# Vandermode/ELD

Measured on AMD Instinct MI355X. Metric: raw megapixels/sec (noise-synth + U-Net step), higher is better.
Workload: dtype f32; 1 GPU; BASELINE.json configs[1]: full ELD noise model (PGRU, SonyA7S2 params) on 4x1424x2128 packed raw + U-Net fp32 train step (fwd, L1, bwd, Adam), 8 frames per GPU; images_per_gpu=8, global_batch=8, parallelism=dp1

## Files before the change

eld_amd/csrc/conv.h:

```cpp
#pragma once
#include "common.h"

typedef float f32x16 __attribute__((ext_vector_type(16)));
typedef float f32x2 __attribute__((ext_vector_type(2)));
typedef __bf16 bf16x2_hw __attribute__((ext_vector_type(2)));

enum ConvMode { CONV_3X3 = 0, CONV_1X1 = 1, CONV_GATHER2X2 = 2 };
enum ConvEpi { EPI_FWD = 0, EPI_CONVT_FWD = 1, EPI_GRAD = 2 };

typedef unsigned short bf16_t;
enum ConvDtype { DT_F32 = 0, DT_BF16 = 1 };

struct ConvArgs {
    const void* in0;
    const void* in1;
    int C0, C1;
    const void* wp;
    int N, H, W;
    int Nout;
    int epi;
    const float* bias;
    int lrelu;
    void* out0;
    void* out1;
// ... 148 lines not shown
__device__ __forceinline__ void eld_wait_vmcnt() { asm volatile("s_waitcnt vmcnt(%0)" ::"n"(N) : "memory"); }
__device__ __forceinline__ void eld_wait_vmcnt_dyn(int n) {
    switch (n) {
#define ELD_W(k) case k: eld_wait_vmcnt<k>(); break;
        ELD_W(1) ELD_W(2) ELD_W(3) ELD_W(4) ELD_W(5) ELD_W(6) ELD_W(7) ELD_W(8) ELD_W(9) ELD_W(10) ELD_W(11) ELD_W(12) ELD_W(13) ELD_W(14) ELD_W(15) ELD_W(16)
        ELD_W(17) ELD_W(18) ELD_W(19) ELD_W(20) ELD_W(21) ELD_W(22) ELD_W(23) ELD_W(24) ELD_W(25) ELD_W(26) ELD_W(27) ELD_W(28) ELD_W(29) ELD_W(30) ELD_W(31) ELD_W(32)
        ELD_W(33) ELD_W(34) ELD_W(35) ELD_W(36) ELD_W(37) ELD_W(38) ELD_W(39) ELD_W(40) ELD_W(41) ELD_W(42) ELD_W(43) ELD_W(44) ELD_W(45) ELD_W(46) ELD_W(47) ELD_W(48)
#undef ELD_W
        default: eld_wait_vmcnt<0>(); break;
    }
}

__device__ __forceinline__ void f32_rows_swap(float4& a, float4& b) {
    auto r = __builtin_amdgcn_permlane16_swap(__float_as_uint(a.x), __float_as_uint(b.x), false, false); a.x = __uint_as_float(r[0]); b.x = __uint_as_float(r[1]);
    r = __builtin_amdgcn_permlane16_swap(__float_as_uint(a.y), __float_as_uint(b.y), false, false); a.y = __uint_as_float(r[0]); b.y = __uint_as_float(r[1]);
    r = __builtin_amdgcn_permlane16_swap(__float_as_uint(a.z), __float_as_uint(b.z), false, false); a.z = __uint_as_float(r[0]); b.z = __uint_as_float(r[1]);
    r = __builtin_amdgcn_permlane16_swap(__float_as_uint(a.w), __float_as_uint(b.w), false, false); a.w = __uint_as_float(r[0]); b.w = __uint_as_float(r[1]);
}
__device__ __forceinline__ void st16(float* p, float4 v, bool wt = false) {
    typedef float f4v __attribute__((ext_vector_type(4)));
    const f4v q = {v.x, v.y, v.z, v.w};
    if (wt) asm volatile("global_store_dwordx4 %0, %1, off sc1" ::"v"(p), "v"(q) : "memory");
    else *reinterpret_cast<float4*>(p) = v;
}
__device__ __forceinline__ void f32_line_store(float4 (&v)[4], float* blk, size_t pstride, int lane, bool row_ok, int valid_px, bool wt = false) {
    f32_rows_swap(v[0], v[1]);
    f32_rows_swap(v[2], v[3]);
    const int lp = lane & 15;
    float* p0 = blk + (size_t)lp * pstride + 4 * bf16_line_group(lane);
    if (row_ok && lp < valid_px) {
        st16(p0, v[0], wt);
        st16(p0 + 16, v[2], wt);
    }
    if (row_ok && lp + 16 < valid_px) {
        float* p1 = p0 + 16 * pstride;
        st16(p1, v[1], wt);
        st16(p1 + 16, v[3], wt);
    }
}

__host__ __device__ inline int vrow_extent(int N, int H, int P) { return (N - 1) * P + H; }
__host__ __device__ inline int vrow_pitch(int N, int H, int TH) {
    const int flat = H + 2 - (H & 1), own = (H + TH - 1) / TH * TH;
    if (flat < TH + 2) return own;
    return (vrow_extent(N, H, flat) + TH - 1) / TH < (vrow_extent(N, H, own) + TH - 1) / TH ? flat : own;
}

void conv_tile_shape(int N, int H, int W, int TH, bool pooled, int& th, int& tw);
__host__ __device__ inline int conv_slot_of_lane(int m, bool grouped) {
    if (!grouped) return m;
    const int q = m >> 2;
    const int sq = q == 0 ? 0 : q == 1 ? 4 : q == 2 ? 5 : q == 3 ? 1 : q == 4 ? 6 : q == 5 ? 2 : q == 6 ? 3 : 7;
    return sq * 4 + (m & 3);
}
__host__ __device__ inline bool conv_slots_grouped(int th, int tw, int TH) { return !(th == TH && tw == 32); }
long long conv_tile_count(int N, int H, int W, int TH, bool pooled);
const char* conv_tile_variant();

__device__ __forceinline__ void f32_line_store2(float4 (&v)[4], float* p0, float* p1, int lane, bool wt = false) {
    f32_rows_swap(v[0], v[1]);
    f32_rows_swap(v[2], v[3]);
    const int g = 4 * bf16_line_group(lane);
    if (p0 != nullptr) {
        st16(p0 + g, v[0], wt);
        st16(p0 + g + 16, v[2], wt);
    }
    if (p1 != nullptr) {
        st16(p1 + g, v[1], wt);
        st16(p1 + g + 16, v[3], wt);
    }
}

int launch_conv(const ConvArgs& a, int mode, hipStream_t st);
int conv_fp32_algo(int set);
inline int resolve_algo(int algo) { return (algo >= 0 && algo <= 2) ? algo : conv_fp32_algo(-1); }
int launch_conv_x3(const ConvArgs& a, hipStream_t st);
int x3_slab_bn(int Nout, int N, int H, int W, int* waves = nullptr);
__host__ __device__ inline size_t x3_slab_stride(int BN) { return (size_t)(3 * BN * 112 + 1023) / 1024 * 1024; }
void conv_x3_set_prof(unsigned long long* buf);
int launch_conv_x3_gemm(const ConvArgs& a, int mode, hipStream_t st);
bool x3w_enabled();
bool x3w_takes(const ConvArgs& a);
int launch_conv_x3w(const ConvArgs& a, hipStream_t st);
int bfd_slab_bn(int Nout, int K, int N, int H, int W);
__host__ __device__ inline size_t bfd_slab_bytes(int BN) { return (size_t)3 * BN * 64; }
int launch_conv_bfd(const ConvArgs& a, hipStream_t st);
int debug_kernel_mask(int set);
bool bfs_takes(int Nout, int K, int N, int H, int W);
int launch_conv_bfs(const ConvArgs& a, hipStream_t st);
bool bfw_takes(const ConvArgs& a);
int launch_conv_bfw(const ConvArgs& a, hipStream_t st);
int bfg_slab_bn(bool gather, int Nout, int Cs, int Cout_t, int N, int H, int W);
__host__ __device__ inline size_t bfg_slab_bytes(int BN) { return (size_t)BN * 64; }
int launch_conv_bfg(const ConvArgs& a, int mode, hipStream_t st);

#ifdef __HIPCC__
__device__ __forceinline__ int xcd_block(int on) {
    const int b = (int)blockIdx.x;
    if (!on) return b;
    const int n = (int)gridDim.x, q = n >> 3, r = n & 7, x = b & 7;
    return (x < r ? x * (q + 1) : r * (q + 1) + (x - r) * q) + (b >> 3);
}
#endif
__host__ __device__ inline void band_tile(int id, int tiles_x, int tiles_y, int BH, int& ty, int& tx) {
    if (BH <= 1) { ty = id / tiles_x; tx = id - ty * tiles_x; return; }
    const int full = tiles_x * BH, band = id / full, off = id - band * full;
    int bh = tiles_y - band * BH;
    if (bh > BH) bh = BH;
    tx = off / bh;
    ty = band * BH + (off - tx * bh);
}
int eld_tile_band();
enum { XCD_GEMM = 1, XCD_WGRAD8 = 2, XCD_WGRAD = 4, XCD_X3D = 8, XCD_X3W = 16, XCD_BF16 = 32, XCD_IGEMM = 64 };
int eld_xcd_mask();

struct WgradArgs {
    const void* g;
    int CA;
    const void* x0;
    const void* x1;
    int C0, C1;
    int N, H, W;
    float* part;
    float* bpart;
    float* xbpart;
    int CBp;
    int psplit;
    int tiles_x, tiles_y;
    int vp;
    int dtype;
    int algo;
    int wgrad8;
    int xcd;
    int band;
    const float* amax_g; const float* amax_x0; const float* amax_x1;
};

int launch_wgrad(const WgradArgs& a, int mode, hipStream_t st);
bool wgrad8_shape(int CA, int CBp, int& COB, int& JB, int& TH, int& TWo, bool bf16 = false);
int wgrad8_ntiles(int CA, int CBp, int N, int H, int W, bool bf16);
bool wgradt8_takes(int CA, int CB);
int wgradt8_ntiles(int N, int H, int W);
int launch_wgrad_reduce(const float* part, const float* bpart, float* wgrad, float* bgrad, int psplit, int T, int CA,
                        int CBp, int CBr, hipStream_t st, int bias_n = 0);
```

eld_amd/csrc/conv_x3.hip:

```cpp
#include <stdlib.h>
#include "conv.h"

#include "conv_x3_dev.h"

namespace {

template <int BN, int RPW, bool DB, bool BFIRST = false, bool BSLAB = false, bool STREAM = false>
__global__ __launch_bounds__(256, 2) void conv_x3_kernel(const ConvArgs a) {
    constexpr int CK = 16;
    constexpr int TH = 4 * RPW, NT = BN / 32, A_PIX = (TH + 2) * (TW + 2);
    constexpr int A_WORDS = A_PIX * PX, B_ROWS = 3 * BN;
    extern __shared__ __attribute__((aligned(16))) float lds[];
    float* ldsA = lds;
    float* ldsB = lds + A_WORDS;

    const int tid = threadIdx.x, lane = tid & 63, wave = tid >> 6;
    const int m = lane & 31, hi = lane >> 5;
    const int NB = a.Nout / BN;
    const int Cin = a.C0 + a.C1;
    const int total_tiles = a.tiles_x * a.tiles_y * a.N * NB;
    const int Cs0 = a.C0;

    constexpr int A_UNITS = A_PIX * 4, B_UNITS = BSLAB ? B_ROWS * 7 : B_ROWS * 4;
    constexpr int A_IT = (A_UNITS + 255) / 256, B_IT = (B_UNITS + 255) / 256;
// ... 813 lines not shown
    }
}

template <bool POOL>
__global__ __launch_bounds__(256) void x3_splitk_finish_kernel(const ConvArgs a) {
    const int Q = a.Nout >> 2;
    const int Wb = POOL ? a.W >> 1 : a.W, Hb = POOL ? a.H >> 1 : a.H;
    const size_t total = (size_t)a.N * Hb * Wb * Q;
    const size_t plane = (size_t)a.N * a.H * a.W * a.Nout;
    for (size_t i = (size_t)blockIdx.x * 256 + threadIdx.x; i < total; i += (size_t)gridDim.x * 256) {
        const int q = (int)(i % Q);
        size_t p = i / Q;
        const int xb = (int)(p % Wb); p /= Wb;
        const int yb = (int)(p % Hb);
        const int img = (int)(p / Hb);
        const int n = 4 * q;
        float4 pooled = make_float4(0.f, 0.f, 0.f, 0.f);
#pragma unroll
        for (int w = 0; w < (POOL ? 4 : 1); ++w) {
            const int y = POOL ? 2 * yb + (w >> 1) : yb, x = POOL ? 2 * xb + (w & 1) : xb;
            const size_t pix = (size_t)(img * a.H + y) * a.W + x;
            float4 v = make_float4(0.f, 0.f, 0.f, 0.f);
            for (int ks = 0; ks < a.ksplit; ++ks) {
                const float4 t = *reinterpret_cast<const float4*>(a.kpart + (size_t)ks * plane + pix * a.Nout + n);
                v.x += t.x; v.y += t.y; v.z += t.z; v.w += t.w;
            }
            if (a.epi == EPI_FWD) {
                const float4 b = *reinterpret_cast<const float4*>(a.bias + n);
                v.x += b.x; v.y += b.y; v.z += b.z; v.w += b.w;
                if (a.lrelu) { v.x = fmaxf(0.2f * v.x, v.x); v.y = fmaxf(0.2f * v.y, v.y); v.z = fmaxf(0.2f * v.z, v.z); v.w = fmaxf(0.2f * v.w, v.w); }
                *reinterpret_cast<float4*>(static_cast<float*>(a.out0) + pix * a.Nout + n) = v;
                if (POOL) pooled = w == 0 ? v : make_float4(fmaxf(pooled.x, v.x), fmaxf(pooled.y, v.y), fmaxf(pooled.z, v.z), fmaxf(pooled.w, v.w));
            } else {
                const bool lo = n < a.split;
                const int C = lo ? a.split : a.Nout - a.split;
                const size_t idx = pix * C + (lo ? n : n - a.split);
                const float* act = static_cast<const float*>(lo ? a.act0 : a.act1);
                if (act) {
                    const float4 s_ = *reinterpret_cast<const float4*>(act + idx);
                    v.x *= lrelu_slope(s_.x); v.y *= lrelu_slope(s_.y); v.z *= lrelu_slope(s_.z); v.w *= lrelu_slope(s_.w);
                }
                *reinterpret_cast<float4*>(static_cast<float*>(lo ? a.out0 : a.out1) + idx) = v;
            }
        }
        if (POOL) *reinterpret_cast<float4*>(static_cast<float*>(a.pool_out) + ((size_t)(img * Hb + yb) * Wb + xb) * a.Nout + n) = pooled;
    }
}

int launch_x3_splitk_finish(const ConvArgs& a, hipStream_t st) {
    const bool pool = a.epi == EPI_FWD && a.pool_out != nullptr;
    const size_t total = (size_t)a.N * (pool ? a.H / 2 : a.H) * (pool ? a.W / 2 : a.W) * (a.Nout / 4);
    if (!total) return 0;
    const unsigned grid = (unsigned)((total + 255) / 256 < 4096 ? (total + 255) / 256 : 4096);
    if (pool) { ELD_LAUNCH(x3_splitk_finish_kernel<true>, dim3(grid), dim3(256), 0, st, a); }
    else { ELD_LAUNCH(x3_splitk_finish_kernel<false>, dim3(grid), dim3(256), 0, st, a); }
    ELD_LAUNCH_CHECK();
    return 0;
}

template <int BN, int RPW, bool DB, bool BFIRST = false, bool BSLAB = false, bool STREAM = false>
int launch_x3(ConvArgs a, hipStream_t st) {
    a.xcd = eld_xcd_mask() & XCD_X3W;
    constexpr int TH = 4 * RPW;
    a.tiles_x = (a.W + TW - 1) / TW;
    a.tiles_y = (a.H + TH - 1) / TH;
    const size_t lds_bytes = (size_t)((TH + 2) * (TW + 2) + 3 * BN) * PX * sizeof(float);
    const long long tiles = (long long)a.tiles_x * a.tiles_y * a.N * (a.Nout / BN);
    if (tiles <= 0) return 0;
    if (tiles > 0x7fffffffLL) return ELD_ENOTSUP;
    eld_note_conv_variant("conv_x3<32>", BSLAB ? nullptr : "cut", BFIRST ? nullptr : "bfirst0", STREAM ? nullptr : "stream0");
    auto kern = conv_x3_kernel<BN, RPW, DB, BFIRST, BSLAB, STREAM>;
    static EldAttrOnce once;
    { const int rc = once.ensure(kern, lds_bytes); if (rc) return rc; }
    int per_cu = (int)((160 * 1024) / lds_bytes);
    if (per_cu > 2) per_cu = 2;
    if (per_cu < 1 || (ELD_DBG(a) & 64)) per_cu = 1;
    long long grid = (long long)eld_num_cus() * per_cu;
    if (grid > tiles) grid = tiles;
    ELD_LAUNCH(kern, dim3((unsigned)grid), dim3(256), lds_bytes, st, a);
    ELD_LAUNCH_CHECK();
    return 0;
}

template <int BN, int RPW, int WAVES, bool DB, int STREAM = 0>
int launch_x3d(ConvArgs a, hipStream_t st) {
    a.xcd = eld_xcd_mask() & XCD_X3D;
    constexpr int TH = WAVES * RPW;
    conv_tile_shape(a.N, a.H, a.W, TH, a.pool_out != nullptr, a.tile_h, a.tile_w);
    a.vp = vrow_pitch(a.N, a.H, a.tile_h);
    a.tiles_x = (a.W + a.tile_w - 1) / a.tile_w;
    a.tiles_y = (vrow_extent(a.N, a.H, a.vp) + a.tile_h - 1) / a.tile_h;
    const size_t lds_bytes = (size_t)(TH + 2) * (TW + 2) * PX * sizeof(float) + 2 * (size_t)((3 * BN * PX * 4 + 1023) / 1024 * 1024);
    long long tiles = (long long)a.tiles_x * a.tiles_y * (a.Nout / BN);
    if (tiles <= 0) return 0;
    a.ksplit = 1;
    static const int no_splitk = [] { const char* e = getenv("ELD_NO_SPLITK"); return e ? atoi(e) : 0; }();
    if (WAVES == 4 && a.kpart != nullptr && !no_splitk) {
        const int nch = (a.C0 + a.C1) / 16;
        const size_t plane = (size_t)a.N * a.H * a.W * a.Nout;
        int ks = (int)(eld_num_cus() / tiles);
        if (ks > nch / 2) ks = nch / 2;
        if (ks > 16) ks = 16;
        while (ks > 1 && (size_t)ks * plane > a.kpart_floats) --ks;
        if (ks >= 2) { a.ksplit = ks; tiles *= ks; }
    }
    if (tiles > 0x7fffffffLL) return ELD_ENOTSUP;
    eld_note_conv_variant(BN == 128 ? "conv_x3d<128,8>" : (BN == 32 ? "conv_x3d<32,8>" : (WAVES == 8 ? "conv_x3d<64,8>" : (a.ksplit > 1 ? "conv_x3d<64,4,splitk>" : "conv_x3d<64,4>"))),
                          (WAVES == 8 && BN >= 64) ? (STREAM == 0 ? "stream0" : (STREAM == 1 ? "wreuse0" : nullptr)) : nullptr,
                          a.pool_out ? nullptr : conv_tile_variant());
    auto kern = conv_x3d_kernel<BN, RPW, WAVES, DB, STREAM>;
    static EldAttrOnce once;
    { const int rc = once.ensure(kern, lds_bytes); if (rc) return rc; }
    int per_cu = (int)((160 * 1024) / lds_bytes);
    if (per_cu > 2) per_cu = 2;
    if (per_cu < 1) per_cu = 1;
    long long grid = (long long)eld_num_cus() * per_cu;
    if (grid > tiles) grid = tiles;
    ELD_LAUNCH(kern, dim3((unsigned)grid), dim3(64 * WAVES), lds_bytes, st, a);
    ELD_LAUNCH_CHECK();
    if (a.ksplit > 1) return launch_x3_splitk_finish(a, st);
    return 0;
}

template <int MODE, int BN, int WAVES>
int launch_x3_gemm(ConvArgs a, hipStream_t st) {
    a.xcd = eld_xcd_mask() & XCD_GEMM;
    constexpr int TH = 2 * WAVES;
    a.tiles_x = (a.W + TW - 1) / TW;
    a.tiles_y = (a.H + TH - 1) / TH;
    const size_t lds_bytes = (size_t)(2 * TH * TW + 2 * BN) * PX * sizeof(float);
    const long long tiles = (long long)a.tiles_x * a.tiles_y * a.N * (a.Nout / BN);
    if (tiles <= 0) return 0;
    if (tiles > 0x7fffffffLL) return ELD_ENOTSUP;
    int per_cu = (int)((160 * 1024) / lds_bytes);
    if (per_cu > 2) per_cu = 2;
    long long grid = (long long)eld_num_cus() * per_cu;
    if (grid > tiles) grid = tiles;
    eld_note_conv_kernel(MODE == CONV_1X1 ? "conv_x3_gemm<1x1>" : "conv_x3_gemm<gather>");
    auto kern = conv_x3_gemm_kernel<MODE, BN, WAVES>;
    static EldAttrOnce once;
    { const int rc = once.ensure(kern, lds_bytes); if (rc) return rc; }
    ELD_LAUNCH(kern, dim3((unsigned)grid), dim3(64 * WAVES), lds_bytes, st, a);
    ELD_LAUNCH_CHECK();
    return 0;
}

}


static bool x3_32_slabs() {
    static const int on = [] { const char* e = getenv("ELD_X3_BSLAB"); return e ? atoi(e) : 0; }();
    return on != 0 || x3w_enabled();
}
static bool x3d_32_kernel(int N, int H, int W) {
    static const int on = [] { const char* e = getenv("ELD_X3D_32"); return e ? atoi(e) : 0; }();
    return on && x3_32_slabs() && conv_tile_count(N, H, W, 32, false) >= 2 * eld_num_cus();
}

int x3_slab_bn(int Nout, int N, int H, int W, int* waves) {
    if (waves) *waves = 8;
    if (Nout == 32) {
        return x3_32_slabs() ? 32 : 0;
    }
    if (Nout % 64) return 0;
    const long long px_tiles = conv_tile_count(N, H, W, 16, false);
    const int cus = eld_num_cus();
    if (Nout % 128 == 0 && px_tiles * (Nout / 128) >= cus) return 128;
    if (waves && px_tiles * (Nout / 64) < cus) *waves = 4;
    return 64;
}

int eld_xcd_mask() {
    static const int m = [] { const char* e = getenv("ELD_XCD"); return e ? atoi(e) : 127; }();
    return m;
}

int eld_tile_band() {
    static const int b = [] { const char* e = getenv("ELD_TILE_BAND"); return e ? atoi(e) : 4; }();
    return b;
}

int launch_conv_x3(const ConvArgs& a_in, hipStream_t st) {
    ConvArgs a = a_in;
    a.prof = nullptr;
    if ((size_t)a.H * a.W * a.C0 * 4 >= 0xFFFFFFF0ull) return ELD_ENOTSUP;
    if (a.pool_out && (a.epi != EPI_FWD || (a.H & 1) || (a.W & 1))) return ELD_EINVAL;
    int waves = 8;
    const int bn0 = x3_slab_bn(a.Nout, a.N, a.H, a.W, nullptr);
    if ((bn0 >= 64 || (bn0 == 32 && x3d_32_kernel(a.N, a.H, a.W))) && a.N > 1 && (size_t)a.H * a.W * a.C0 * 8 >= 0xFFFFFFF0ull) return ELD_ENOTSUP;
    const int bn = x3_slab_bn(a.Nout, a.N, a.H, a.W, &waves);
    static const int stream = [] { const char* e = getenv("ELD_X3_STREAM"); return e ? atoi(e) : 7; }();
    if (bn == 32 && x3w_takes(a)) return launch_conv_x3w(a, st);
    if (bn == 32 && x3d_32_kernel(a.N, a.H, a.W)) return launch_x3d<32, 4, 8, false>(a, st);
    if (bn == 32) return (stream & 1) ? launch_x3<32, 4, false, true, true, true>(a, st) : launch_x3<32, 4, false, true, true>(a, st);
    static const int wreuse = [] { const char* e = getenv("ELD_X3_WREUSE"); return e ? atoi(e) : 6; }();
    if (bn == 128) {
        if ((stream & 4) && (wreuse & 4)) return launch_x3d<128, 2, 8, false, 2>(a, st);
        return (stream & 4) ? launch_x3d<128, 2, 8, false, 1>(a, st) : launch_x3d<128, 2, 8, false>(a, st);
    }
    if (bn == 64) {
        if (waves != 8) return launch_x3d<64, 2, 4, false>(a, st);
        if ((stream & 2) && (wreuse & 2)) return launch_x3d<64, 2, 8, false, 2>(a, st);
        return (stream & 2) ? launch_x3d<64, 2, 8, false, 1>(a, st) : launch_x3d<64, 2, 8, false>(a, st);
    }
    static const int bfirst = [] { const char* e = getenv("ELD_X3_BFIRST"); return e ? atoi(e) : 1; }();
    if (bfirst) return (stream & 1) ? launch_x3<32, 4, false, true, false, true>(a, st) : launch_x3<32, 4, false, true>(a, st);
    return launch_x3<32, 4, false>(a, st);
}

int launch_conv_x3_gemm(const ConvArgs& a, int mode, hipStream_t st) {
    const size_t src_img = (size_t)a.H * a.W * a.C0 * 4 * (mode == CONV_GATHER2X2 ? 4 : 1);
    if (a.Nout % 64 || a.C0 % 32 || a.C1 != 0 || src_img >= 0xFFFFFFF0ull) return ELD_ENOTSUP;
    if (mode == CONV_1X1 && a.epi == EPI_CONVT_FWD && a.Cout_t % 32) return ELD_ENOTSUP;
    if (mode == CONV_1X1 && a.epi == EPI_CONVT_FWD) return launch_x3_gemm<CONV_1X1, 64, 4>(a, st);
    if (mode == CONV_GATHER2X2 && a.epi == EPI_GRAD && a.split == a.Nout) return launch_x3_gemm<CONV_GATHER2X2, 64, 4>(a, st);
    return ELD_ENOTSUP;
}
```

eld_amd/csrc/conv_x3w.hip:

```cpp
#include <stdlib.h>
#include <type_traits>
#include "conv_x3_dev.h"

namespace {

template <int N>
__device__ __forceinline__ void w_wait_vm() { asm volatile("s_waitcnt vmcnt(%0)" ::"n"(N) : "memory"); }

struct WProf {
    unsigned long long* p; int n;
    __device__ __forceinline__ void operator()(unsigned tag) {
        if (p != nullptr && n < 1024) { p[n] = ((unsigned long long)tag << 56) | (__builtin_readcyclecounter() & 0x00FFFFFFFFFFFFFFull); ++n; }
    }
};

constexpr int W_BN = 32, W_TH = 16, W_CK = 16;
constexpr int W_APIX = (W_TH + 2) * (TW + 2);
constexpr int W_AWORDS = W_APIX * PX;
constexpr int W_BROWS = 3 * W_BN;
constexpr int W_BWORDS = (W_BROWS * PX * 4 + 1023) / 1024 * 256;
constexpr int W_BPIECES = W_BWORDS * 4 / 1024;
constexpr int W_AUNITS = W_APIX * 4;

template <int W_CW, int W_RPW, bool SLABW, bool PRIO, int W_PW = 4, bool PAIR = false>
__global__ __launch_bounds__(64 * (W_CW + W_PW), (W_CW + W_PW) / 4) void conv_x3w_kernel(const ConvArgs a) {
    static_assert(W_CW * W_RPW == W_TH, "tile rows");
    static_assert(!PAIR || SLABW, "paired halo loads: the halo waves wait for nothing but their own loads");
    constexpr int W_HW = SLABW ? W_PW - 1 : W_PW;
    constexpr int W_PTHREADS = 64 * W_HW;
    constexpr int W_AIT = (W_AUNITS + W_PTHREADS - 1) / W_PTHREADS;
    constexpr int W_T0 = (W_AIT + 2) / 3, W_T1 = W_T0 + (W_AIT - W_T0 + 1) / 2;
    extern __shared__ __attribute__((aligned(16))) float lds[];
    float* ldsB = lds;
    float* ldsA = lds + 2 * W_BWORDS;
    const int tid = threadIdx.x, lane = tid & 63;
    const int wave = __builtin_amdgcn_readfirstlane(tid >> 6);
    const bool consumer = wave < W_CW;
    const int m = lane & 31, hi = lane >> 5;
    const int Cin = a.C0 + a.C1, NCH = Cin / W_CK;
    const int tiles_img = a.tiles_x * a.tiles_y;
    const int total_tiles = tiles_img * a.N;
    const int first = xcd_block(a.xcd), stride = gridDim.x;
    if (first >= total_tiles) return;
    const int my_tiles = (total_tiles - first + stride - 1) / stride;
    const int n_chunks = my_tiles * NCH;

    auto decode = [&](int t, int& img, int& y0, int& x0) {
        img = t / tiles_img;
        const int r = t - img * tiles_img;
        int ty, tx;
        band_tile(r, a.tiles_x, a.tiles_y, a.band, ty, tx);
        y0 = ty * W_TH; x0 = tx * TW;
    };

    unsigned long long* prof_base = ELD_PROF(a);
    const int prole = wave == 0 ? 0 : (wave == W_CW ? 1 : (wave == W_CW + W_PW - 1 ? 2 : -1));
    WProf prof = {(prof_base != nullptr && blockIdx.x < 8 && prole >= 0 && lane == 0) ? prof_base + ((size_t)blockIdx.x * 3 + prole) * 1024 : nullptr, 0};
    const unsigned ldsB_addr = (unsigned)__builtin_amdgcn_readfirstlane((int)(size_t)(__attribute__((address_space(3))) float*)ldsB);
    const unsigned long long wbase = (unsigned long long)a.wp;
    const i32x4 rsrc_w = {(int)(unsigned)wbase, (int)((unsigned)(wbase >> 32) & 0xFFFFu), (int)((size_t)3 * NCH * W_BWORDS * 4), 0x00020000};
    using I0_ = std::integral_constant<int, 0>;
    using I1_ = std::integral_constant<int, 1>;
    using IA_ = std::integral_constant<int, W_T0>;
    using IB_ = std::integral_constant<int, W_T1>;
    using IE_ = std::integral_constant<int, W_AIT>;

    auto dma_slab = [&](int buf, int c, int ky) {
        const unsigned soff = (unsigned)((ky * NCH + c) * (W_BWORDS * 4));
        constexpr int MOVERS = SLABW ? 1 : W_PW;
        const int first_piece = SLABW ? 0 : wave - W_CW;
#pragma unroll
        for (int it = 0; it < (W_BPIECES + MOVERS - 1) / MOVERS; ++it) {
            const int piece = first_piece + it * MOVERS;
            if (piece < W_BPIECES) bdma16(rsrc_w, (unsigned)lane * 16u, soff + (unsigned)(piece * 1024), ldsB_addr + (unsigned)(buf * W_BWORDS * 4 + piece * 1024));
        }
    };

    if (SLABW && wave == W_CW + W_HW) {
        if constexpr (PRIO) __builtin_amdgcn_s_setprio(3);
        dma_slab(0, 0, 0);
        dma_wait();
        __syncthreads();
        int g = 0, sb = 0;
        for (int k = 0; k < my_tiles; ++k)
            for (int c = 0; c < NCH; ++c) {
                for (int ky = 0; ky < 3; ++ky) {
                    int c1 = c, ky1 = ky + 1;
                    if (ky1 == 3) { ky1 = 0; c1 = c + 1 < NCH ? c + 1 : 0; }
                    prof(20);
                    if (g + 1 < n_chunks || ky < 2) dma_slab(sb ^ 1, c1, ky1);
                    prof(21);
                    dma_wait();
                    prof(22);
                    __syncthreads();
                    sb ^= 1;
                }
                ++g;
            }
        return;
    }
    if (!consumer) {
        if constexpr (PRIO) __builtin_amdgcn_s_setprio(3);
        const int ptid = tid - 64 * W_CW;
        constexpr unsigned OOB = 0xFFFFFFF0u;
        float4 ra[2][W_AIT];
        unsigned a_voff[2][W_AIT];
        int s_img[2] = {0, 0}, s_tile[2] = {-1, -1};
        auto setup_set = [&](auto S, int t) {
            constexpr int s = decltype(S)::value;
            int y0, x0;
// ... 7 lines not shown
                const int gy = y0 + hy - 1, gx = x0 + hx - 1;
                const bool ok = u < W_AUNITS && gy >= 0 && gy < a.H && gx >= 0 && gx < a.W;
                a_voff[s][it] = ok ? (unsigned)(gy * a.W + gx) * (unsigned)(a.C0 * 4) + (unsigned)part * 16u : OOB;
            }
        };
        auto load_part = [&](auto S, auto I0, auto I1, int g) {
            constexpr int s = decltype(S)::value;
            if (g >= n_chunks) return;
            const int t = first + (g / NCH) * stride, c = g % NCH;
            if (t != s_tile[s]) setup_set(S, t);
            const int c0 = c * W_CK;
            const char* src = static_cast<const char*>(c0 < a.C0 ? a.in0 : a.in1);
            const int cs = c0 < a.C0 ? c0 : c0 - a.C0;
            const size_t img_bytes = (size_t)a.H * a.W * a.C0 * 4;
            const __amdgpu_buffer_rsrc_t rsrc_a = __builtin_amdgcn_make_buffer_rsrc((void*)(src + (size_t)s_img[s] * img_bytes), 0, (int)img_bytes, 0x00020000);
#pragma unroll
            for (int it = decltype(I0)::value; it < decltype(I1)::value; ++it)
                ra[s][it] = __builtin_bit_cast(float4, __builtin_amdgcn_raw_buffer_load_b128(rsrc_a, (int)a_voff[s][it], cs * 4, 0));
        };
        auto cut_part = [&](auto S, auto I0, auto I1) {
            constexpr int s = decltype(S)::value;
#pragma unroll
            for (int it = decltype(I0)::value; it < decltype(I1)::value; ++it) {
                const int u = ptid + it * W_PTHREADS;
                if (u < W_AUNITS) split_store(ldsA + s * W_AWORDS + stage_row(u >> 2, W_APIX) * PX + (u & 3) * 2, ra[s][it]);
            }
        };
        if constexpr (!SLABW) dma_slab(0, 0, 0);
        load_part(I0_{}, I0_{}, IE_{}, 0);
        load_part(I1_{}, I0_{}, IE_{}, 1);
        cut_part(I0_{}, I0_{}, IE_{});
        if constexpr (!PAIR) load_part(I0_{}, I0_{}, IE_{}, 2);
        __syncthreads();
        int g = 0, sb = 0;
        for (int k = 0; k < my_tiles; ++k) {
            for (int cp = 0; cp < NCH; cp += 2) {
                auto chunk = [&](auto SN, int c) {
#pragma unroll
                    for (int ky = 0; ky < 3; ++ky) {
                        if constexpr (!SLABW) {
                            int c1 = c, ky1 = ky + 1;
                            if (ky1 == 3) { ky1 = 0; c1 = c + 1 < NCH ? c + 1 : 0; }
                            if (g + 1 < n_chunks || ky < 2) dma_slab(sb ^ 1, c1, ky1);
                        }
                        prof(10);
                        if constexpr (PAIR) {
                            constexpr bool even = decltype(SN)::value == 1;
                            using SO = std::integral_constant<int, 1 - decltype(SN)::value>;
                            if (g + 1 < n_chunks) {
                                if (ky == 0) cut_part(SN, I0_{}, IA_{}); else if (ky == 1) cut_part(SN, IA_{}, IB_{}); else cut_part(SN, IB_{}, IE_{});
                            }
                            prof(11);
                            if constexpr (even) {
                                if (ky == 0) { load_part(SO{}, I0_{}, IA_{}, g + 2); load_part(SN, I0_{}, IA_{}, g + 3); }
                                else if (ky == 1) { load_part(SO{}, IA_{}, IB_{}, g + 2); load_part(SN, IA_{}, IB_{}, g + 3); }
                                else { load_part(SO{}, IB_{}, IE_{}, g + 2); load_part(SN, IB_{}, IE_{}, g + 3); }
                            }
                        } else
                        if (g + 1 < n_chunks) {
                            if (ky == 0) { cut_part(SN, I0_{}, IA_{}); prof(11); load_part(SN, I0_{}, IA_{}, g + 3); }
                            else if (ky == 1) { cut_part(SN, IA_{}, IB_{}); prof(11); load_part(SN, IA_{}, IB_{}, g + 3); }
                            else { cut_part(SN, IB_{}, IE_{}); prof(11); load_part(SN, IB_{}, IE_{}, g + 3); }
                        }
                        prof(12);
                        if constexpr (!SLABW) {
                            if (g + 3 < n_chunks) {
                                if (ky == 0) w_wait_vm<W_T0>(); else if (ky == 1) w_wait_vm<W_T1 - W_T0>(); else w_wait_vm<W_AIT - W_T1>();
                            } else dma_wait();
                        }
                        prof(13);
                        __syncthreads();
                        sb ^= 1;
                    }
                    ++g;
                };
                chunk(I1_{}, cp);
                chunk(I0_{}, cp + 1);
            }
        }
        return;
    }

    __syncthreads();
    f32x16 acc[W_RPW][1];
    int sb = 0;
    int g = 0;
    for (int k = 0; k < my_tiles; ++k) {
        const int t = first + k * stride;
#pragma unroll
        for (int r = 0; r < W_RPW; ++r)
#pragma unroll
            for (int i = 0; i < 16; ++i) acc[r][0][i] = 0.f;
        for (int c = 0; c < NCH; ++c) {
            const float* la = ldsA + (c & 1) * W_AWORDS;
#pragma unroll
            for (int ky = 0; ky < 3; ++ky) {
                const float* lb = ldsB + sb * W_BWORDS;
                prof(1);
                x3_stage_blocks<W_RPW, 1>(acc,
                    [&](int kx, int r, uint4 (&X)[3]) {
                        const float* p = la + ((wave * W_RPW + r + ky) * (TW + 2) + m + kx) * PX + hi * 4;
#pragma unroll
                        for (int pc = 0; pc < 3; ++pc) X[pc] = *reinterpret_cast<const uint4*>(p + pc * 8);
                    },
                    [&](int kx, int tt, uint4 (&Wt)[3]) {
                        const float* p = lb + (kx * W_BN + m) * PX + hi * 4;
#pragma unroll
                        for (int pc = 0; pc < 3; ++pc) Wt[pc] = *reinterpret_cast<const uint4*>(p + pc * 8);
                    });
                prof(2);
                __syncthreads();
                sb ^= 1;
            }
            ++g;
        }

        prof(3);
        int img, y0, x0;
        decode(t, img, y0, x0);
        constexpr int RPW = W_RPW, NT = 1, BN = W_BN;
        const int nb = 0;
        {
            const int x = x0 + m;
            const bool xok = x < a.W;
            if (a.epi == EPI_FWD) {
                const float sl = a.lrelu ? 0.2f : 1.0f;
#pragma unroll
                for (int q = 0; q < 4; ++q) {
                    const float4 bq = *reinterpret_cast<const float4*>(a.bias + 4 * hi + 8 * q);
#pragma unroll
                    for (int r = 0; r < RPW; ++r) bias_lrelu4(acc[r][0], 4 * q, bq, sl);
                }
                if (a.codes_out != nullptr && xok) {
#pragma unroll
                    for (int r = 0; r < RPW; ++r) {
                        const int y = y0 + wave * RPW + r;
                        if (y >= a.H) continue;
                        const size_t pix = (size_t)(img * a.H + y) * a.W + x;
                        a.codes_out[pix * 2 + hi] = slope_codes16(acc[r][0]);
                    }
                }
            }
            unsigned cw[RPW];
            if (a.epi != EPI_FWD && a.codes0 != nullptr) {
#pragma unroll
                for (int r = 0; r < RPW; ++r) {
                    const int y = y0 + wave * RPW + r;
                    const size_t pix = (size_t)(img * a.H + (y < a.H ? y : 0)) * a.W + (xok ? x : 0);
                    cw[r] = a.codes0[pix * 2 + hi];
                }
            }
#pragma unroll
            for (int r = 0; r < RPW; ++r) {
                const int y = y0 + wave * RPW + r;
                const bool yok = y < a.H;
                const size_t rowpix = (size_t)(img * a.H + (yok ? y : 0)) * a.W;
                const size_t pix = rowpix + (xok ? x : 0);
                float4 v[4];
#pragma unroll
                for (int q = 0; q < 4; ++q) v[q] = make_float4(acc[r][0][4 * q], acc[r][0][4 * q + 1], acc[r][0][4 * q + 2], acc[r][0][4 * q + 3]);
                float* blk = static_cast<float*>(a.out0) + (rowpix + x0) * BN;
                if (a.epi != EPI_FWD) {
                    const float* act = static_cast<const float*>(a.act0);
                    if (a.codes0 != nullptr) {
                        const unsigned w = cw[r];
#pragma unroll
                        for (int q = 0; q < 4; ++q) {
                            v[q].x *= slope_of_code(w, 4 * q); v[q].y *= slope_of_code(w, 4 * q + 1);
                            v[q].z *= slope_of_code(w, 4 * q + 2); v[q].w *= slope_of_code(w, 4 * q + 3);
                        }
                    } else if (act != nullptr) {
                        float4 s[4];
#pragma unroll
                        for (int q = 0; q < 4; ++q) s[q] = *reinterpret_cast<const float4*>(act + pix * BN + 4 * hi + 8 * q);
#pragma unroll
                        for (int q = 0; q < 4; ++q) {
                            v[q].x *= lrelu_slope(s[q].x); v[q].y *= lrelu_slope(s[q].y);
                            v[q].z *= lrelu_slope(s[q].z); v[q].w *= lrelu_slope(s[q].w);
                        }
                    }
                }
                f32_line_store(v, blk, (size_t)BN, lane, yok, a.W - x0);
            }
        }
        if (a.epi == EPI_FWD && a.pool_out != nullptr) {
            int img_p[RPW / 2], y_p[RPW / 2];
#pragma unroll
            for (int rp = 0; rp < RPW / 2; ++rp) { img_p[rp] = img; y_p[rp] = y0 + wave * RPW + 2 * rp; }
            pool_epilogue<RPW, NT, BN>(a, acc, img_p, nb, y_p, x0 + m, hi);
        }
        prof(4);
    }
}

}

static int x3w_mode() {
    static const int on = [] { const char* e = getenv("ELD_X3W"); return e ? atoi(e) : 5; }();
    return on;
}
bool x3w_enabled() { return x3w_mode() != 0; }
bool x3w_takes(const ConvArgs& a) {
    if (!x3w_enabled() || a.Nout != 32 || a.dtype != DT_F32) return false;
    const int Cin = a.C0 + a.C1;
    if ((Cin != 32 && Cin != 64) || a.C0 % 32) return false;
    if (a.epi == EPI_GRAD && (a.split != 32 || a.out1 != nullptr || a.act1 != nullptr || a.codes1 != nullptr)) return false;
    if (a.epi != EPI_FWD && a.epi != EPI_GRAD) return false;
    const long long tiles = (long long)((a.W + TW - 1) / TW) * ((a.H + W_TH - 1) / W_TH) * a.N;
    return tiles >= eld_num_cus();
}

static unsigned long long* g_x3w_prof = nullptr;
void conv_x3_set_prof(unsigned long long* buf) { g_x3w_prof = buf; }

int launch_conv_x3w(const ConvArgs& a_in, hipStream_t st) {
    ConvArgs a = a_in;
    a.xcd = eld_xcd_mask() & XCD_X3W;
    a.band = eld_tile_band();
    a.prof = ELD_DEV_TOOLS ? g_x3w_prof : nullptr;
    a.tiles_x = (a.W + TW - 1) / TW;
    a.tiles_y = (a.H + W_TH - 1) / W_TH;
    const long long tiles = (long long)a.tiles_x * a.tiles_y * a.N;
    if (tiles <= 0) return 0;
    if (tiles > 0x3fffffffLL) return ELD_ENOTSUP;
    constexpr size_t lds_bytes = (size_t)(2 * W_BWORDS + 2 * W_AWORDS) * sizeof(float);
    long long grid = (long long)eld_num_cus();
    if (grid > tiles) grid = tiles;
    const int mode = x3w_mode();
    eld_note_conv_variant("conv_x3w", mode == 5 ? nullptr : (mode == 7 ? "m7" : (mode == 4 ? "m4" : (mode == 1 ? "m1" : (mode == 3 ? "m3" : "m2")))));
    if (mode == 7) {
        static EldAttrOnce once;
        { const int rc = once.ensure(conv_x3w_kernel<8, 2, true, false, 8, true>, lds_bytes); if (rc) return rc; }
        ELD_LAUNCH((conv_x3w_kernel<8, 2, true, false, 8, true>), dim3((unsigned)grid), dim3(1024), lds_bytes, st, a);
    } else if (mode == 5) {
        static EldAttrOnce once;
        { const int rc = once.ensure(conv_x3w_kernel<8, 2, true, false, 8>, lds_bytes); if (rc) return rc; }
        ELD_LAUNCH((conv_x3w_kernel<8, 2, true, false, 8>), dim3((unsigned)grid), dim3(1024), lds_bytes, st, a);
    } else if (mode == 4) {
        static EldAttrOnce once;
        { const int rc = once.ensure(conv_x3w_kernel<8, 2, false, false, 8>, lds_bytes); if (rc) return rc; }
        ELD_LAUNCH((conv_x3w_kernel<8, 2, false, false, 8>), dim3((unsigned)grid), dim3(1024), lds_bytes, st, a);
    } else if (mode == 1) {
        static EldAttrOnce once;
        { const int rc = once.ensure(conv_x3w_kernel<4, 4, true, false>, lds_bytes); if (rc) return rc; }
        ELD_LAUNCH((conv_x3w_kernel<4, 4, true, false>), dim3((unsigned)grid), dim3(512), lds_bytes, st, a);
    } else if (mode == 3) {
        static EldAttrOnce once;
        { const int rc = once.ensure(conv_x3w_kernel<8, 2, false, true>, lds_bytes); if (rc) return rc; }
        ELD_LAUNCH((conv_x3w_kernel<8, 2, false, true>), dim3((unsigned)grid), dim3(768), lds_bytes, st, a);
    } else {
        static EldAttrOnce once;
        { const int rc = once.ensure(conv_x3w_kernel<8, 2, false, false>, lds_bytes); if (rc) return rc; }
        ELD_LAUNCH((conv_x3w_kernel<8, 2, false, false>), dim3((unsigned)grid), dim3(768), lds_bytes, st, a);
    }
    ELD_LAUNCH_CHECK();
    return 0;
}
```

Before: 726.4 raw MPix/s.

## Extend warp-specialized x3w conv kernel to 64 output channels and route 64-wide convs

Generalizes the conv_x3w kernel geometry with a template for tile height and number of 32-channel output blocks, allowing a 64-output-channel variant with split output/codes handling for gradient epilogues. The 64-channel 8-wave streaming path now dispatches to this new x3w64 kernel when enough tiles exist, instead of the x3d kernel. The aim is to reuse each loaded input halo across twice as many output channels with the producer/consumer wave structure of x3w. It adds register pressure and a new epilogue path for split outputs, and changes the tile shape to 12 rows.

After: 732.1 raw MPix/s, median of 6. About the same (+0.8%).

```diff
diff --git a/eld_amd/csrc/conv.h b/eld_amd/csrc/conv.h
--- a/eld_amd/csrc/conv.h
+++ b/eld_amd/csrc/conv.h
@@ -254,6 +254,8 @@
 bool x3w_enabled();
 bool x3w_takes(const ConvArgs& a);
 int launch_conv_x3w(const ConvArgs& a, hipStream_t st);
+bool x3w64_takes(const ConvArgs& a);
+int launch_conv_x3w64(const ConvArgs& a, hipStream_t st);
 int bfd_slab_bn(int Nout, int K, int N, int H, int W);
 __host__ __device__ inline size_t bfd_slab_bytes(int BN) { return (size_t)3 * BN * 64; }
 int launch_conv_bfd(const ConvArgs& a, hipStream_t st);
diff --git a/eld_amd/csrc/conv_x3.hip b/eld_amd/csrc/conv_x3.hip
--- a/eld_amd/csrc/conv_x3.hip
+++ b/eld_amd/csrc/conv_x3.hip
@@ -919,6 +919,18 @@
     return 0;
 }
 
+int x3d_ksplit(const ConvArgs& a, long long tiles) {
+    static const int no_splitk = [] { const char* e = getenv("ELD_NO_SPLITK"); return e ? atoi(e) : 0; }();
+    if (a.kpart == nullptr || no_splitk) return 1;
+    const int nch = (a.C0 + a.C1) / 16;
+    const size_t plane = (size_t)a.N * a.H * a.W * a.Nout;
+    int ks = (int)(eld_num_cus() / tiles);
+    if (ks > nch / 2) ks = nch / 2;
+    if (ks > 16) ks = 16;
+    while (ks > 1 && (size_t)ks * plane > a.kpart_floats) --ks;
+    return ks >= 2 ? ks : 1;
+}
+
 template <int BN, int RPW, int WAVES, bool DB, int STREAM = 0>
 int launch_x3d(ConvArgs a, hipStream_t st) {
     a.xcd = eld_xcd_mask() & XCD_X3D;
@@ -930,17 +942,8 @@
     const size_t lds_bytes = (size_t)(TH + 2) * (TW + 2) * PX * sizeof(float) + 2 * (size_t)((3 * BN * PX * 4 + 1023) / 1024 * 1024);
     long long tiles = (long long)a.tiles_x * a.tiles_y * (a.Nout / BN);
     if (tiles <= 0) return 0;
-    a.ksplit = 1;
-    static const int no_splitk = [] { const char* e = getenv("ELD_NO_SPLITK"); return e ? atoi(e) : 0; }();
-    if (WAVES == 4 && a.kpart != nullptr && !no_splitk) {
-        const int nch = (a.C0 + a.C1) / 16;
-        const size_t plane = (size_t)a.N * a.H * a.W * a.Nout;
-        int ks = (int)(eld_num_cus() / tiles);
-        if (ks > nch / 2) ks = nch / 2;
-        if (ks > 16) ks = 16;
-        while (ks > 1 && (size_t)ks * plane > a.kpart_floats) --ks;
-        if (ks >= 2) { a.ksplit = ks; tiles *= ks; }
-    }
+    a.ksplit = WAVES == 4 ? x3d_ksplit(a, tiles) : 1;
+    tiles *= a.ksplit;
     if (tiles > 0x7fffffffLL) return ELD_ENOTSUP;
     eld_note_conv_variant(BN == 128 ? "conv_x3d<128,8>" : (BN == 32 ? "conv_x3d<32,8>" : (WAVES == 8 ? "conv_x3d<64,8>" : (a.ksplit > 1 ? "conv_x3d<64,4,splitk>" : "conv_x3d<64,4>"))),
                           (WAVES == 8 && BN >= 64) ? (STREAM == 0 ? "stream0" : (STREAM == 1 ? "wreuse0" : nullptr)) : nullptr,
@@ -1036,8 +1039,12 @@
         return (stream & 4) ? launch_x3d<128, 2, 8, false, 1>(a, st) : launch_x3d<128, 2, 8, false>(a, st);
     }
     if (bn == 64) {
-        if (waves != 8) return launch_x3d<64, 2, 4, false>(a, st);
-        if ((stream & 2) && (wreuse & 2)) return launch_x3d<64, 2, 8, false, 2>(a, st);
+        if (waves != 8) {
+            if ((debug_kernel_mask(-1) & 512) && x3w64_takes(a) && x3d_ksplit(a, conv_tile_count(a.N, a.H, a.W, 8, a.pool_out != nullptr) * (a.Nout / 64)) == 1)
+                return launch_conv_x3w64(a, st);
+            return launch_x3d<64, 2, 4, false>(a, st);
+        }
+        if ((stream & 2) && (wreuse & 2)) return x3w64_takes(a) ? launch_conv_x3w64(a, st) : launch_x3d<64, 2, 8, false, 2>(a, st);
         return (stream & 2) ? launch_x3d<64, 2, 8, false, 1>(a, st) : launch_x3d<64, 2, 8, false>(a, st);
     }
     static const int bfirst = [] { const char* e = getenv("ELD_X3_BFIRST"); return e ? atoi(e) : 1; }();
diff --git a/eld_amd/csrc/conv_x3w.hip b/eld_amd/csrc/conv_x3w.hip
--- a/eld_amd/csrc/conv_x3w.hip
+++ b/eld_amd/csrc/conv_x3w.hip
@@ -14,18 +14,23 @@
     }
 };
 
-constexpr int W_BN = 32, W_TH = 16, W_CK = 16;
-constexpr int W_APIX = (W_TH + 2) * (TW + 2);
-constexpr int W_AWORDS = W_APIX * PX;
-constexpr int W_BROWS = 3 * W_BN;
-constexpr int W_BWORDS = (W_BROWS * PX * 4 + 1023) / 1024 * 256;
-constexpr int W_BPIECES = W_BWORDS * 4 / 1024;
-constexpr int W_AUNITS = W_APIX * 4;
-
-template <int W_CW, int W_RPW, bool SLABW, bool PRIO, int W_PW = 4, bool PAIR = false>
+constexpr int W_CK = 16;
+template <int TH, int NT>
+struct WGeom {
+    static constexpr int BN = 32 * NT;
+    static constexpr int APIX = (TH + 2) * (TW + 2);
+    static constexpr int AWORDS = APIX * PX;
+    static constexpr int BWORDS = (3 * BN * PX * 4 + 1023) / 1024 * 256;
+    static constexpr int BPIECES = BWORDS * 4 / 1024;
+    static constexpr int AUNITS = APIX * 4;
+    static constexpr size_t LDS_BYTES = (size_t)(2 * BWORDS + 2 * AWORDS) * sizeof(float);
+};
+
+template <int W_CW, int W_RPW, bool SLABW, bool PRIO, int W_PW = 4, bool PAIR = false, int W_NT = 1>
 __global__ __launch_bounds__(64 * (W_CW + W_PW), (W_CW + W_PW) / 4) void conv_x3w_kernel(const ConvArgs a) {
-    static_assert(W_CW * W_RPW == W_TH, "tile rows");
     static_assert(!PAIR || SLABW, "paired halo loads: the halo waves wait for nothing but their own loads");
+    using Geom = WGeom<W_CW * W_RPW, W_NT>;
+    constexpr int W_TH = W_CW * W_RPW, W_BN = Geom::BN, W_APIX = Geom::APIX, W_AWORDS = Geom::AWORDS, W_BWORDS = Geom::BWORDS, W_BPIECES = Geom::BPIECES, W_AUNITS = Geom::AUNITS;
     constexpr int W_HW = SLABW ? W_PW - 1 : W_PW;
     constexpr int W_PTHREADS = 64 * W_HW;
     constexpr int W_AIT = (W_AUNITS + W_PTHREADS - 1) / W_PTHREADS;
@@ -199,7 +204,7 @@
     }
 
     __syncthreads();
-    f32x16 acc[W_RPW][1];
+    f32x16 acc[W_RPW][W_NT];
     int sb = 0;
     int g = 0;
     for (int k = 0; k < my_tiles; ++k) {
@@ -207,21 +212,23 @@
 #pragma unroll
         for (int r = 0; r < W_RPW; ++r)
 #pragma unroll
-            for (int i = 0; i < 16; ++i) acc[r][0][i] = 0.f;
+            for (int tt = 0; tt < W_NT; ++tt)
+#pragma unroll
+                for (int i = 0; i < 16; ++i) acc[r][tt][i] = 0.f;
         for (int c = 0; c < NCH; ++c) {
             const float* la = ldsA + (c & 1) * W_AWORDS;
 #pragma unroll
             for (int ky = 0; ky < 3; ++ky) {
                 const float* lb = ldsB + sb * W_BWORDS;
                 prof(1);
-                x3_stage_blocks<W_RPW, 1>(acc,
+                x3_stage_blocks<W_RPW, W_NT, (W_RPW > 1 && W_NT > 1)>(acc,
                     [&](int kx, int r, uint4 (&X)[3]) {
                         const float* p = la + ((wave * W_RPW + r + ky) * (TW + 2) + m + kx) * PX + hi * 4;
 #pragma unroll
                         for (int pc = 0; pc < 3; ++pc) X[pc] = *reinterpret_cast<const uint4*>(p + pc * 8);
                     },
                     [&](int kx, int tt, uint4 (&Wt)[3]) {
-                        const float* p = lb + (kx * W_BN + m) * PX + hi * 4;
+                        const float* p = lb + (kx * W_BN + tt * 32 + m) * PX + hi * 4;
 #pragma unroll
                         for (int pc = 0; pc < 3; ++pc) Wt[pc] = *reinterpret_cast<const uint4*>(p + pc * 8);
                     });
@@ -235,36 +242,50 @@
         prof(3);
         int img, y0, x0;
         decode(t, img, y0, x0);
-        constexpr int RPW = W_RPW, NT = 1, BN = W_BN;
-        const int nb = 0;
+        constexpr int RPW = W_RPW, NT = W_NT, BN = W_BN;
+        auto block_dest = [&](int tt, bool& lo, int& C, int& cb) {
+            if (NT == 1 || a.epi == EPI_FWD) { lo = true; C = BN; cb = tt * 32; return; }
+            lo = tt * 32 < a.split;
+            C = lo ? a.split : BN - a.split;
+            cb = lo ? tt * 32 : tt * 32 - a.split;
+        };
         {
             const int x = x0 + m;
             const bool xok = x < a.W;
             if (a.epi == EPI_FWD) {
                 const float sl = a.lrelu ? 0.2f : 1.0f;
 #pragma unroll
-                for (int q = 0; q < 4; ++q) {
-                    const float4 bq = *reinterpret_cast<const float4*>(a.bias + 4 * hi + 8 * q);
-#pragma unroll
-                    for (int r = 0; r < RPW; ++r) bias_lrelu4(acc[r][0], 4 * q, bq, sl);
-                }
+                for (int tt = 0; tt < NT; ++tt)
+#pragma unroll
+                    for (int q = 0; q < 4; ++q) {
+                        const float4 bq = *reinterpret_cast<const float4*>(a.bias + tt * 32 + 4 * hi + 8 * q);
+#pragma unroll
+                        for (int r = 0; r < RPW; ++r) bias_lrelu4(acc[r][tt], 4 * q, bq, sl);
+                    }
                 if (a.codes_out != nullptr && xok) {
 #pragma unroll
                     for (int r = 0; r < RPW; ++r) {
                         const int y = y0 + wave * RPW + r;
                         if (y >= a.H) continue;
                         const size_t pix = (size_t)(img * a.H + y) * a.W + x;
-                        a.codes_out[pix * 2 + hi] = slope_codes16(acc[r][0]);
+#pragma unroll
+                        for (int tt = 0; tt < NT; ++tt) a.codes_out[(pix * NT + tt) * 2 + hi] = slope_codes16(acc[r][tt]);
                     }
                 }
             }
-            unsigned cw[RPW];
-            if (a.epi != EPI_FWD && a.codes0 != nullptr) {
+            unsigned cw[RPW][NT];
+            if (a.epi != EPI_FWD && (a.codes0 != nullptr || (NT > 1 && a.codes1 != nullptr))) {
 #pragma unroll
                 for (int r = 0; r < RPW; ++r) {
                     const int y = y0 + wave * RPW + r;
                     const size_t pix = (size_t)(img * a.H + (y < a.H ? y : 0)) * a.W + (xok ? x : 0);
-                    cw[r] = a.codes0[pix * 2 + hi];
+#pragma unroll
+                    for (int tt = 0; tt < NT; ++tt) {
+                        bool lo; int C, cb;
+                        block_dest(tt, lo, C, cb);
+                        const unsigned* cd = lo ? a.codes0 : a.codes1;
+                        cw[r][tt] = cd != nullptr ? cd[(pix * (size_t)(C >> 5) + (size_t)(cb >> 5)) * 2 + hi] : 0u;
+                    }
                 }
             }
 #pragma unroll
@@ -273,38 +294,45 @@
                 const bool yok = y < a.H;
                 const size_t rowpix = (size_t)(img * a.H + (yok ? y : 0)) * a.W;
                 const size_t pix = rowpix + (xok ? x : 0);
-                float4 v[4];
-#pragma unroll
-                for (int q = 0; q < 4; ++q) v[q] = make_float4(acc[r][0][4 * q], acc[r][0][4 * q + 1], acc[r][0][4 * q + 2], acc[r][0][4 * q + 3]);
-                float* blk = static_cast<float*>(a.out0) + (rowpix + x0) * BN;
-                if (a.epi != EPI_FWD) {
-                    const float* act = static_cast<const float*>(a.act0);
-                    if (a.codes0 != nullptr) {
-                        const unsigned w = cw[r];
-#pragma unroll
-                        for (int q = 0; q < 4; ++q) {
-                            v[q].x *= slope_of_code(w, 4 * q); v[q].y *= slope_of_code(w, 4 * q + 1);
-                            v[q].z *= slope_of_code(w, 4 * q + 2); v[q].w *= slope_of_code(w, 4 * q + 3);
-                        }
-                    } else if (act != nullptr) {
-                        float4 s[4];
-#pragma unroll
-                        for (int q = 0; q < 4; ++q) s[q] = *reinterpret_cast<const float4*>(act + pix * BN + 4 * hi + 8 * q);
-#pragma unroll
-                        for (int q = 0; q < 4; ++q) {
-                            v[q].x *= lrelu_slope(s[q].x); v[q].y *= lrelu_slope(s[q].y);
-                            v[q].z *= lrelu_slope(s[q].z); v[q].w *= lrelu_slope(s[q].w);
+#pragma unroll
+                for (int tt = 0; tt < NT; ++tt) {
+                    float4 v[4];
+#pragma unroll
+                    for (int q = 0; q < 4; ++q) v[q] = make_float4(acc[r][tt][4 * q], acc[r][tt][4 * q + 1], acc[r][tt][4 * q + 2], acc[r][tt][4 * q + 3]);
+                    bool lo; int C, cb;
+                    block_dest(tt, lo, C, cb);
+                    float* blk = static_cast<float*>(lo ? a.out0 : a.out1) + (rowpix + x0) * C + cb;
+                    if (a.epi != EPI_FWD) {
+                        const float* act = static_cast<const float*>(lo ? a.act0 : a.act1);
+                        if ((lo ? a.codes0 : a.codes1) != nullptr) {
+                            const unsigned w = cw[r][tt];
+#pragma unroll
+                            for (int q = 0; q < 4; ++q) {
+                                v[q].x *= slope_of_code(w, 4 * q); v[q].y *= slope_of_code(w, 4 * q + 1);
+                                v[q].z *= slope_of_code(w, 4 * q + 2); v[q].w *= slope_of_code(w, 4 * q + 3);
+                            }
+                        } else if (act != nullptr) {
+                            float4 s[4];
+#pragma unroll
+                            for (int q = 0; q < 4; ++q) s[q] = *reinterpret_cast<const float4*>(act + pix * C + cb + 4 * hi + 8 * q);
+#pragma unroll
+                            for (int q = 0; q < 4; ++q) {
+                                v[q].x *= lrelu_slope(s[q].x); v[q].y *= lrelu_slope(s[q].y);
+                                v[q].z *= lrelu_slope(s[q].z); v[q].w *= lrelu_slope(s[q].w);
+                            }
                         }
                     }
+                    f32_line_store(v, blk, (size_t)C, lane, yok, a.W - x0);
                 }
-                f32_line_store(v, blk, (size_t)BN, lane, yok, a.W - x0);
             }
         }
-        if (a.epi == EPI_FWD && a.pool_out != nullptr) {
-            int img_p[RPW / 2], y_p[RPW / 2];
-#pragma unroll
-            for (int rp = 0; rp < RPW / 2; ++rp) { img_p[rp] = img; y_p[rp] = y0 + wave * RPW + 2 * rp; }
-            pool_epilogue<RPW, NT, BN>(a, acc, img_p, nb, y_p, x0 + m, hi);
+        if constexpr (RPW % 2 == 0) {
+            if (a.epi == EPI_FWD && a.pool_out != nullptr) {
+                int img_p[RPW / 2], y_p[RPW / 2];
+#pragma unroll
+                for (int rp = 0; rp < RPW / 2; ++rp) { img_p[rp] = img; y_p[rp] = y0 + wave * RPW + 2 * rp; }
+                pool_epilogue<RPW, NT, BN>(a, acc, img_p, 0, y_p, x0 + m, hi);
+            }
         }
         prof(4);
     }
@@ -323,26 +351,64 @@
     if ((Cin != 32 && Cin != 64) || a.C0 % 32) return false;
     if (a.epi == EPI_GRAD && (a.split != 32 || a.out1 != nullptr || a.act1 != nullptr || a.codes1 != nullptr)) return false;
     if (a.epi != EPI_FWD && a.epi != EPI_GRAD) return false;
-    const long long tiles = (long long)((a.W + TW - 1) / TW) * ((a.H + W_TH - 1) / W_TH) * a.N;
+    if ((size_t)a.H * a.W * a.C0 * 4 >= 0xFFFFFFF0ull) return false;
+    const long long tiles = (long long)((a.W + TW - 1) / TW) * ((a.H + 15) / 16) * a.N;
     return tiles >= eld_num_cus();
+}
+
+constexpr int X3W64_TH = 12, X3W64_MIN_TILES_PER_CU = 8;
+bool x3w64_takes(const ConvArgs& a) {
+    const int mask = debug_kernel_mask(-1);
+    if (!x3w_enabled() || (mask & 1024) || a.Nout != 64 || a.dtype != DT_F32) return false;
+    const int Cin = a.C0 + a.C1;
+    if (Cin % 32 || a.C0 % 32 || (a.C1 != 0 && a.C1 != a.C0)) return false;
+    if (a.epi == EPI_FWD) { if (a.pool_out != nullptr || a.pool_codes_out != nullptr) return false; }
+    else if (a.epi == EPI_GRAD) { if (a.split != 64 && (a.split != 32 || a.out1 == nullptr)) return false; }
+    else return false;
+    if ((size_t)a.H * a.W * a.C0 * 4 >= 0xFFFFFFF0ull) return false;
+    const long long tiles = (long long)((a.W + TW - 1) / TW) * ((a.H + X3W64_TH - 1) / X3W64_TH) * a.N;
+    if (mask & 512) return tiles > 0;
+    return tiles >= (long long)X3W64_MIN_TILES_PER_CU * eld_num_cus();
 }
 
 static unsigned long long* g_x3w_prof = nullptr;
 void conv_x3_set_prof(unsigned long long* buf) { g_x3w_prof = buf; }
 
-int launch_conv_x3w(const ConvArgs& a_in, hipStream_t st) {
-    ConvArgs a = a_in;
+static int x3w_prepare(ConvArgs& a, int TH, long long& grid) {
     a.xcd = eld_xcd_mask() & XCD_X3W;
     a.band = eld_tile_band();
     a.prof = ELD_DEV_TOOLS ? g_x3w_prof : nullptr;
     a.tiles_x = (a.W + TW - 1) / TW;
-    a.tiles_y = (a.H + W_TH - 1) / W_TH;
+    a.tiles_y = (a.H + TH - 1) / TH;
     const long long tiles = (long long)a.tiles_x * a.tiles_y * a.N;
-    if (tiles <= 0) return 0;
-    if (tiles > 0x3fffffffLL) return ELD_ENOTSUP;
-    constexpr size_t lds_bytes = (size_t)(2 * W_BWORDS + 2 * W_AWORDS) * sizeof(float);
-    long long grid = (long long)eld_num_cus();
-    if (grid > tiles) grid = tiles;
+    grid = tiles < (long long)eld_num_cus() ? tiles : (long long)eld_num_cus();
+    return tiles > 0x3fffffffLL ? ELD_ENOTSUP : 0;
+}
+
+template <int CW, int RPW, int PW>
+static int launch_x3w64(ConvArgs a, const char* variant, hipStream_t st) {
+    long long grid;
+    { const int rc = x3w_prepare(a, CW * RPW, grid); if (rc) return rc; }
+    if (grid <= 0) return 0;
+    constexpr size_t lds_bytes = WGeom<CW * RPW, 2>::LDS_BYTES;
+    eld_note_conv_variant("conv_x3w64", variant);
+    static EldAttrOnce once;
+    { const int rc = once.ensure(conv_x3w_kernel<CW, RPW, true, false, PW, false, 2>, lds_bytes); if (rc) return rc; }
+    ELD_LAUNCH((conv_x3w_kernel<CW, RPW, true, false, PW, false, 2>), dim3((unsigned)grid), dim3(64 * (CW + PW)), lds_bytes, st, a);
+    ELD_LAUNCH_CHECK();
+    return 0;
+}
+int launch_conv_x3w64(const ConvArgs& a, hipStream_t st) {
+    if (debug_kernel_mask(-1) & 2048) return launch_x3w64<8, 1, 8>(a, "c8", st);
+    return launch_x3w64<X3W64_TH / 3, 3, 4>(a, nullptr, st);
+}
+
+int launch_conv_x3w(const ConvArgs& a_in, hipStream_t st) {
+    ConvArgs a = a_in;
+    long long grid;
+    { const int rc = x3w_prepare(a, 16, grid); if (rc) return rc; }
+    if (grid <= 0) return 0;
+    constexpr size_t lds_bytes = WGeom<16, 1>::LDS_BYTES;
     const int mode = x3w_mode();
     eld_note_conv_variant("conv_x3w", mode == 5 ? nullptr : (mode == 7 ? "m7" : (mode == 4 ? "m4" : (mode == 1 ? "m1" : (mode == 3 ? "m3" : "m2")))));
     if (mode == 7) {
```
